# lab-incert/peba1

Measured on AMD Instinct MI355X. Metric: bootstrapped gates/sec (blind rotations/s) over the PEBA1 match path, and end-to-end match ms, higher is better.
Workload: dtype u32

## Files before the change

peba1_amd/csrc/kernels.hip:

```cpp
#include <type_traits>

#include "kernels.hpp"
#include "ntt_wave.hpp"

namespace tfhe_hip {

namespace {

__device__ __forceinline__ PrimeCtx make_ctx(int q, const uint32_t *tw, int n_ring) {
    PrimeCtx c;
    c.P = q ? NTT_P1 : NTT_P0;
    c.pinv = q ? NTT_PINV1 : NTT_PINV0;
    c.rmod = q ? NTT_R[1] : NTT_R[0];
    c.wf = tw + (size_t)(q * 2 + 0) * n_ring;
    c.wi = tw + (size_t)(q * 2 + 1) * n_ring;
    const uint4 *quads = reinterpret_cast<const uint4 *>(tw + (size_t)4 * n_ring);
    c.qf = quads + (size_t)(q * 2 + 0) * (n_ring / 2);
    c.qi = quads + (size_t)(q * 2 + 1) * (n_ring / 2);
    c.dtab = nullptr;
    c.fw1 = nullptr;
    c.fw2 = nullptr;
    return c;
}

__device__ __forceinline__ PrimeCtx make_sub_ctx(int q, int h, const uint32_t *tw, int n_ring) {
    return make_ctx(q, tw + (size_t)12 * n_ring + (size_t)h * 6 * n_ring, n_ring / 2);
}

template <int LOGN>
__device__ __forceinline__ void finish_inverse(const int64_t (&acc)[WaveNtt<LOGN>::REGS],
                                               int32_t (&y)[WaveNtt<LOGN>::REGS],
                                               const PrimeCtx &c, uint32_t *scr, int lane) {
    constexpr int REGS = WaveNtt<LOGN>::REGS;
#pragma unroll
    for (int r = 0; r < REGS; ++r) y[r] = mont_redc(acc[r], c.P, c.pinv);
    WaveNtt<LOGN>::inverse(y, c, scr, lane);
}

template <int LOGN>
__global__ __launch_bounds__(64) void bk_transform_kernel(const int32_t *__restrict__ raw, uint32_t *__restrict__ img,
                                                          const uint32_t *__restrict__ tw, int nw,
                                                          uint32_t scale0, uint32_t scale1) {
    using NTT = WaveNtt<LOGN>;
    constexpr int N = NTT::N, REGS = NTT::REGS;
    __shared__ __align__(16) uint32_t scr[NTT::SCRATCH_WORDS];
    const int lane = threadIdx.x;
    const int q = blockIdx.y;
    const int poly = blockIdx.x;
    const int X = poly / nw, w = poly % nw;
    const PrimeCtx c = make_ctx(q, tw, N);
    const uint32_t scale = q ? scale1 : scale0;
    const int32_t *src = raw + (size_t)poly * N;
    int32_t x[REGS];
#pragma unroll
    for (int r = 0; r < REGS; ++r) x[r] = src[r * 64 + lane] % (int32_t)c.P;
    NTT::forward(x, c, scr, lane);
    uint4 *dst = reinterpret_cast<uint4 *>(img + ((size_t)(X * 2 + q) * nw + w) * N) + lane;
#pragma unroll
    for (int g = 0; g < REGS / 4; ++g) {
        uint32_t v[4];
#pragma unroll
        for (int e = 0; e < 4; ++e) {
            int32_t m = x[4 * g + e] % (int32_t)c.P;
            if (m < 0) m += (int32_t)c.P;
            v[e] = (uint32_t)((uint64_t)(uint32_t)m * scale % c.P);
        }
        dst[g * 64] = make_uint4(v[0], v[1], v[2], v[3]);
    }
}

template <int LOGN>
__global__ __launch_bounds__(128) void negacyclic_kernel(const int32_t *__restrict__ ip, const uint32_t *__restrict__ img,
                                                         const uint32_t *__restrict__ tw, int32_t *__restrict__ res) {
    using NTT = WaveNtt<LOGN>;
    constexpr int N = NTT::N, REGS = NTT::REGS;
    __shared__ __align__(16) uint32_t lds_scr[2][NTT::SCRATCH_WORDS];
    const int tid = threadIdx.x;
    const int q = __builtin_amdgcn_readfirstlane(tid >> 6);
    const int lane = tid & 63;
    const PrimeCtx c = make_ctx(q, tw, N);
    uint32_t *scr = lds_scr[q];
    const int32_t *src = ip + (size_t)blockIdx.x * N;
    int32_t x[REGS];
#pragma unroll
    for (int r = 0; r < REGS; ++r) x[r] = src[r * 64 + lane];
    NTT::forward(x, c, scr, lane);
    const uint4 *bp = reinterpret_cast<const uint4 *>(img + (size_t)(blockIdx.x * 2 + q) * N) + lane;
    int64_t acc[REGS];
#pragma unroll
    for (int g = 0; g < REGS / 4; ++g) {
        const uint4 b = bp[g * 64];
        acc[4 * g + 0] = (int64_t)x[4 * g + 0] * (int32_t)b.x;
        acc[4 * g + 1] = (int64_t)x[4 * g + 1] * (int32_t)b.y;
        acc[4 * g + 2] = (int64_t)x[4 * g + 2] * (int32_t)b.z;
        acc[4 * g + 3] = (int64_t)x[4 * g + 3] * (int32_t)b.w;
    }
    int32_t y[REGS];
    finish_inverse<LOGN>(acc, y, c, scr, lane);
#pragma unroll
    for (int r = 0; r < REGS; ++r) scr[r * 64 + lane] = (uint32_t)y[r];
    __syncthreads();
    if (q == 0) {
        const uint32_t *oscr = lds_scr[1];
#pragma unroll
        for (int r = 0; r < REGS; ++r)
            res[(size_t)blockIdx.x * N + r * 64 + lane] = (int32_t)crt_signed_to_torus(y[r], (int32_t)oscr[r * 64 + lane]);
    }
}

template <int LOGN, int THREADS>
__device__ __forceinline__ void prelude_modswitch(const DevParams &p, const RotDesc &rd, const int32_t *__restrict__ pool,
                                                  uint16_t *lds_bar, int tid) {
    const int32_t *A = pool + (size_t)rd.slot_a * p.ct_stride;
    const int32_t *B = pool + (size_t)rd.slot_b * p.ct_stride;
    if (rd.slot_c < 0) {
        for (int i = tid; i <= p.n; i += THREADS) {
            uint32_t t = (uint32_t)rd.sa * (uint32_t)A[i] + (uint32_t)rd.sb * (uint32_t)B[i];
            if (i == p.n) t += (uint32_t)rd.c0;
            lds_bar[i] = (uint16_t)((t + (1u << (30 - LOGN))) >> (31 - LOGN));
        }
    } else {
        const int32_t *C = pool + (size_t)rd.slot_c * p.ct_stride;
        for (int i = tid; i <= p.n; i += THREADS) {
            uint32_t t = (uint32_t)rd.sa * (uint32_t)A[i] + (uint32_t)rd.sb * (uint32_t)B[i] + (uint32_t)rd.sc * (uint32_t)C[i];
            if (i == p.n) t += (uint32_t)rd.c0;
            lds_bar[i] = (uint16_t)((t + (1u << (30 - LOGN))) >> (31 - LOGN));
        }
    }
}

struct ClockProbe {
    unsigned long long c0 = 0, r0 = 0;
    bool on = false;
    __device__ __forceinline__ void begin(const DevParams &p) {
        on = p.clock_acc != nullptr && blockIdx.x % 61 == 0 && threadIdx.x == 0;
        if (on) { c0 = __builtin_amdgcn_s_memtime(); r0 = __builtin_amdgcn_s_memrealtime(); }
    }
    __device__ __forceinline__ void end(const DevParams &p) {
        if (on) {
            atomicAdd(&p.clock_acc[0], __builtin_amdgcn_s_memtime() - c0);
            atomicAdd(&p.clock_acc[1], __builtin_amdgcn_s_memrealtime() - r0);
        }
    }
};

template <int LOGN>
__device__ __forceinline__ uint32_t testvector_coef(int j, int barb, int32_t mu) {
    constexpr int N = 1 << LOGN;
    const int idx = (j + barb) & (2 * N - 1);
    return (idx & N) ? (uint32_t)(-mu) : (uint32_t)mu;
}

template <int LOGN>
__device__ __forceinline__ uint32_t lut_coef(const int32_t *__restrict__ v, int j, int barb) {
    constexpr int N = 1 << LOGN;
    const int idx = (j + barb) & (2 * N - 1);
    const uint32_t w = (uint32_t)v[idx & (N - 1)];
    return (idx & N) ? 0u - w : w;
}

__device__ __forceinline__ const int32_t *lut_of(const DevParams &p, const RotDesc &rd) {
    return rd.lut >= 0 ? p.luts + (size_t)rd.lut * LUT_STRIDE : nullptr;
}

template <int LOGN>
__device__ __forceinline__ uint32_t body_coef(const int32_t *__restrict__ lut, int j, int barb, int32_t mu) {
    return lut ? lut_coef<LOGN>(lut, j, barb) : testvector_coef<LOGN>(j, barb, mu);
}

template <int LOGN>
struct AccLds {
    static constexpr int N = 1 << LOGN;
    uint32_t w[2][3 * N];
    __device__ __forceinline__ void set(int u, int j, uint32_t v) {
        w[u][j] = v; w[u][N + j] = 0u - v; w[u][2 * N + j] = v;
    }
    __device__ __forceinline__ uint32_t get(int u, int j) const { return w[u][j]; }
    template <int REGS>
    __device__ __forceinline__ void rotated_difference(uint32_t (&D)[REGS], int u, int lane, int abar, uint32_t offset) const {
        const uint32_t base = (uint32_t)(lane - abar) & (uint32_t)(2 * N - 1);
        const uint32_t *own_neg = w[u] + N + lane;
        const uint32_t *rot = w[u] + base;
#pragma unroll
        for (int r = 0; r < REGS; ++r) D[r] = (rot[r * 64] + own_neg[r * 64] + offset) ^ offset;
    }
};

template <int LOGN, bool FRESH, bool TABLE, bool LDSTW = false, bool PROGRESS = false, int V = 0>
__device__ __forceinline__ void forward_poly(const DevParams &p, const DevKey &key, const PrimeCtx &c,
                                             const AccLds<LOGN> &lds_acc, uint32_t *scr,
                                             int lane, int q, int i, int u, int abar, bool swap_outputs,
                                             int64_t (&acc0)[WaveNtt<LOGN>::REGS], int64_t (&acc1)[WaveNtt<LOGN>::REGS],
                                             const typename WaveNtt<LOGN>::FwdTw0 &t0, int jbegin = 0, int jend = -1) {
    using NTT = WaveNtt<LOGN>;
    constexpr int N = NTT::N, REGS = NTT::REGS, G4 = REGS / 4;
    uint32_t Dk[REGS];
    lds_acc.template rotated_difference<REGS>(Dk, u, lane, abar, p.decomp_offset);
    const int o0 = swap_outputs ? N / 4 : 0, o1 = N / 4 - o0;
    const int width = p.Bgbit;
    auto row = [&](int jj, auto first) {
        const int prow = u * p.l + jj;
        const uint4 *bp = reinterpret_cast<const uint4 *>(
                              key.bk_img + ((size_t)((size_t)i * p.kpl + prow) * 2 + q) * 2 * N) + lane;
        uint4 b0[G4], b1[G4];
#pragma unroll
        for (int g = 0; g < G4; ++g) b0[g] = bp[o0 + g * 64];
#pragma unroll
        for (int g = 0; g < G4; ++g) b1[g] = bp[o1 + g * 64];
        const int shift = 32 - (jj + 1) * width;
        int32_t x[REGS];
        NTT::template forward_digits<TABLE, LDSTW>(x, Dk, shift, width, c, scr, lane, t0);
#pragma unroll
        for (int g = 0; g < G4; ++g) {
            const int32_t bb0[4] = {(int32_t)b0[g].x, (int32_t)b0[g].y, (int32_t)b0[g].z, (int32_t)b0[g].w};
#pragma unroll
            for (int e = 0; e < 4; ++e) {
                const int r = 4 * g + e;
                if constexpr (decltype(first)::value) acc0[r] = (int64_t)x[r] * bb0[e];
                else acc0[r] += (int64_t)x[r] * bb0[e];
            }
        }
#pragma unroll
        for (int g = 0; g < G4; ++g) {
            const int32_t bb1[4] = {(int32_t)b1[g].x, (int32_t)b1[g].y, (int32_t)b1[g].z, (int32_t)b1[g].w};
#pragma unroll
            for (int e = 0; e < 4; ++e) {
                const int r = 4 * g + e;
                if constexpr (decltype(first)::value) acc1[r] = (int64_t)x[r] * bb1[e];
                else acc1[r] += (int64_t)x[r] * bb1[e];
            }
        }
    };
    if (jend < 0) jend = p.l;
    row(jbegin, std::integral_constant<bool, FRESH>{});
#pragma unroll 1
    for (int jj = jbegin + 1; jj < jend; ++jj) {
        if constexpr (PROGRESS) {
            if (jj == jbegin + 1) __builtin_amdgcn_s_setprio(1);
            else __builtin_amdgcn_s_setprio(2);
        }
        row(jj, std::false_type{});
    }
}

template <int LOGN, int THREADS, typename AccT>
__device__ __forceinline__ void extract_sample(const DevParams &p, const RotDesc &rd,
                                               const AccT &acc,
                                               int32_t *__restrict__ u_buf, int32_t *__restrict__ acc_dbg, int tid) {
    constexpr int N = 1 << LOGN;
    int32_t *u = u_buf + (size_t)rd.u_index * p.u_stride;
    for (int j = tid; j < N; j += THREADS)
        u[j] = (int32_t)(j == 0 ? acc.get(0, 0) : 0u - acc.get(0, N - j));
    if (tid == 0) u[N] = (int32_t)acc.get(1, 0);
    if (acc_dbg) {
        int32_t *d = acc_dbg + (size_t)blockIdx.x * 2 * N;
        for (int j = tid; j < 2 * N; j += THREADS) d[j] = (int32_t)acc.get(j >> LOGN, j & (N - 1));
    }
}

template <int LOGN>
__global__ __launch_bounds__(128) void blind_rotate2_kernel(DevParams p, DevKey key, const int32_t *__restrict__ pool,
                                                           const RotDesc *__restrict__ rots,
                                                           int32_t *__restrict__ u_buf, int32_t *__restrict__ acc_dbg) {
    using NTT = WaveNtt<LOGN>;
    constexpr int N = NTT::N, REGS = NTT::REGS;
    __shared__ __align__(16) AccLds<LOGN> lds_acc;
    __shared__ __align__(16) uint32_t lds_scr[2][NTT::SCRATCH_WORDS];
    __shared__ uint16_t lds_bar[1024 + 8];

    const int tid = threadIdx.x;
    const int q = __builtin_amdgcn_readfirstlane(tid >> 6);
    const int lane = tid & 63;
    const PrimeCtx c = make_ctx(q, key.tw, N);
    uint32_t *scr = lds_scr[q];
    const RotDesc rd = rots[blockIdx.x];
    const int n = p.n;

    prelude_modswitch<LOGN, 128>(p, rd, pool, lds_bar, tid);
    __syncthreads();
    {
        const int barb = lds_bar[n];
        const int32_t *lut = lut_of(p, rd);
#pragma unroll
        for (int r = 0; r < REGS; ++r) {
            const int j = r * 64 + lane;
            lds_acc.set(q, j, q == 0 ? 0u : body_coef<LOGN>(lut, j, barb, p.mu));
        }
    }
    __syncthreads();

    typename NTT::FwdTw0 t0;
    t0.load(c, lane);
    for (int i = 0; i < n; ++i) {
        const int abar = __builtin_amdgcn_readfirstlane((int)lds_bar[i]);
        if (abar == 0) continue;

        int64_t acc0[REGS], acc1[REGS];
        forward_poly<LOGN, true, false>(p, key, c, lds_acc, scr, lane, q, i, 0, abar, false, acc0, acc1, t0);
        forward_poly<LOGN, false, false>(p, key, c, lds_acc, scr, lane, q, i, 1, abar, false, acc0, acc1, t0);

        int32_t y0[REGS], y1[REGS];
        finish_inverse<LOGN>(acc0, y0, c, scr, lane);
        finish_inverse<LOGN>(acc1, y1, c, scr, lane);

        const uint32_t *oscr = lds_scr[1 - q];
        if (q == 0) {
#pragma unroll
            for (int r = 0; r < REGS; ++r) scr[r * 64 + lane] = (uint32_t)y1[r];
            __syncthreads();
#pragma unroll
            for (int r = 0; r < REGS; ++r)
                lds_acc.set(0, r * 64 + lane, lds_acc.get(0, r * 64 + lane) + crt_signed_to_torus(y0[r], (int32_t)oscr[r * 64 + lane]));
        } else {
#pragma unroll
            for (int r = 0; r < REGS; ++r) scr[r * 64 + lane] = (uint32_t)y0[r];
            __syncthreads();
#pragma unroll
            for (int r = 0; r < REGS; ++r)
                lds_acc.set(1, r * 64 + lane, lds_acc.get(1, r * 64 + lane) + crt_signed_to_torus((int32_t)oscr[r * 64 + lane], y1[r]));
        }
        __syncthreads();
    }
    extract_sample<LOGN, 128>(p, rd, lds_acc, u_buf, acc_dbg, tid);
}

#ifdef TFHE_HIP_STAMPS
__device__ unsigned long long g_stamps[8][8];
#define STAMP_DECL unsigned long long st_prev = __builtin_amdgcn_s_memtime(), st_sum[8] = {0, 0, 0, 0, 0, 0, 0, 0}
#define STAMP(k)                                                             \
    do {                                                                     \
        __builtin_amdgcn_sched_barrier(0);                                   \
        const unsigned long long st_now = __builtin_amdgcn_s_memtime();      \
        __builtin_amdgcn_s_waitcnt(0xC07F);                                  \
        st_sum[k] += st_now - st_prev;                                       \
        st_prev = st_now;                                                    \
        __builtin_amdgcn_sched_barrier(0);                                   \
    } while (0)
#define STAMP_FLUSH                                                          \
    do {                                                                     \
        if (lane == 0)                                                       \
            for (int k = 0; k < 8; ++k) atomicAdd(&g_stamps[wv][k], st_sum[k]); \
    } while (0)
#else
#define STAMP_DECL
#define STAMP(k)
#define STAMP_FLUSH
#endif

template <int LOGN>
struct Br4Lds {
    using NTT = WaveNtt<LOGN>;
    AccLds<LOGN> acc;
    uint32_t buf0[4][NTT::SCRATCH_WORDS];
    uint32_t buf1[4][NTT::ROW_WORDS];
    uint16_t bar[1024 + 8];
    alignas(8) uint32_t dtab[2][5 * DIGIT_TAB];
    uint4 ft1[2][64 >> NTT::LC][NTT::FwdTw1::IMAGE16];
    uint4 ft2[2][64][NTT::FwdTw2::IMAGE16];
    __device__ __forceinline__ uint32_t *scr(int wv) { return buf0[wv]; }
    __device__ __forceinline__ uint32_t *x1(int wv) { return buf1[wv]; }
    __device__ __forceinline__ uint32_t *x2(int wv) { return buf0[wv]; }
};
static_assert(sizeof(Br4Lds<10>) <= 80 * 1024, "two workgroups of the 4-wave form must fit the 160 KB of a CU");

template <int LOGN, bool TAB, int V = 0>
__device__ __forceinline__ void blind_rotate4_body(const DevParams &p, const DevKey &key,
                                                   const int32_t *__restrict__ pool, const RotDesc &rd,
                                                   Br4Lds<LOGN> &sh, int tid) {
    using NTT = WaveNtt<LOGN>;
    constexpr int N = NTT::N, REGS = NTT::REGS, HALF = REGS / 2;
    const int wv = __builtin_amdgcn_readfirstlane(tid >> 6);
    const int q = wv & 1, u = wv >> 1;
    const int lane = tid & 63;
    PrimeCtx c = make_ctx(q, key.tw, N);
    uint32_t *scr = sh.scr(wv);
    const int n = p.n;

    prelude_modswitch<LOGN, 256>(p, rd, pool, sh.bar, tid);
    if constexpr (TAB) {
        NTT::build_digit_table(sh.dtab[q], c, p.Bgbit, (u << 6) | lane, 128);
        c.dtab = sh.dtab[q];
    }
    if (u == 0) {
        typename NTT::FwdTw1 a;
        a.load(c, lane);
        if ((lane & ((1 << NTT::LC) - 1)) == 0) a.to_image(sh.ft1[q][lane >> NTT::LC]);
        typename NTT::FwdTw2 b;
        b.load(c, lane);
        b.to_image(sh.ft2[q][lane]);
    }
    c.fw1 = sh.ft1[q][lane >> NTT::LC];
    c.fw2 = sh.ft2[q][lane];
    __syncthreads();
    if (q == 0) {
        const int barb = sh.bar[n];
        const int32_t *lut = lut_of(p, rd);
#pragma unroll
        for (int r = 0; r < REGS; ++r) {
            const int j = r * 64 + lane;
            sh.acc.set(u, j, u == 0 ? 0u : body_coef<LOGN>(lut, j, barb, p.mu));
        }
    }
    __syncthreads();

    STAMP_DECL;
    typename NTT::FwdTw0 t0;
    t0.load(c, lane);

    for (int i = 0; i < n; ++i) {
        const int abar = __builtin_amdgcn_readfirstlane((int)sh.bar[i]);
        if (abar == 0) continue;
        STAMP(0);

        int64_t acc0[REGS], acc1[REGS];
        forward_poly<LOGN, true, TAB, true, true, V>(p, key, c, sh.acc, scr, lane, q, i, u, abar, u != 0, acc0, acc1, t0);
        STAMP(1);

        int32_t t[REGS];
        {
            int32_t send[REGS];
#pragma unroll
            for (int r = 0; r < REGS; ++r) {
                t[r] = mont_redc(acc0[r], c.P, c.pinv);
                send[r] = mont_redc(acc1[r], c.P, c.pinv);
            }
            NTT::write_row(send, sh.x1(wv), lane);
        }
        typename NTT::InvTw2 t2;
        t2.load(c, lane);
        STAMP(2);
        lds_barrier();
        __builtin_amdgcn_s_setprio(3);
        STAMP(3);
        {
            int32_t other[REGS];
            NTT::read_row(other, sh.x1(wv ^ 2), lane);
#pragma unroll
            for (int r = 0; r < REGS; ++r) t[r] += other[r];
        }
        NTT::inverse(t, c, scr, lane, t2);
        STAMP(4);

        const uint32_t *ox = sh.x2(wv ^ 1);
        uint32_t *mx = sh.x2(wv);
        if (q == 0) {
#pragma unroll
            for (int r = 0; r < HALF; ++r) mx[r * 64 + lane] = (uint32_t)t[HALF + r];
            LDS_BARRIER_ROLE("q=0");
#pragma unroll
            for (int r = 0; r < HALF; ++r)
                sh.acc.set(u, r * 64 + lane, sh.acc.get(u, r * 64 + lane) + crt_signed_to_torus(t[r], (int32_t)ox[r * 64 + lane]));
        } else {
#pragma unroll
            for (int r = 0; r < HALF; ++r) mx[r * 64 + lane] = (uint32_t)t[r];
            LDS_BARRIER_ROLE("q=1");
#pragma unroll
            for (int r = 0; r < HALF; ++r)
                sh.acc.set(u, (HALF + r) * 64 + lane,
                           sh.acc.get(u, (HALF + r) * 64 + lane) + crt_signed_to_torus((int32_t)ox[r * 64 + lane], t[HALF + r]));
        }
        STAMP(5);
        __builtin_amdgcn_s_setprio(0);
        lds_barrier();
        STAMP(6);
    }
    STAMP_FLUSH;
}

template <int LOGN, bool TAB>
__global__ __launch_bounds__(256, 2) void blind_rotate4_kernel(
    DevParams p, DevKey key, const int32_t *__restrict__ pool, const RotDesc *__restrict__ rots,
    int32_t *__restrict__ u_buf, int32_t *__restrict__ acc_dbg) {
    __shared__ __align__(16) Br4Lds<LOGN> sh;
    if (p.wg_times && threadIdx.x == 0) {
        const uint64_t hw = __builtin_amdgcn_s_getreg((31 << 11) | (0 << 6) | 4);
        const uint64_t xcc = __builtin_amdgcn_s_getreg((3 << 11) | (0 << 6) | 20);
        p.wg_times[4 * blockIdx.x] = (__builtin_amdgcn_s_memtime() & 0xFFFFFFFFFFFFull) |
                                     ((((xcc & 0xF) << 8) | ((hw >> 8) & 0xFF)) << 48);
        p.wg_times[4 * blockIdx.x + 2] = __builtin_amdgcn_s_memrealtime();
    }
    ClockProbe clk;
    clk.begin(p);
    const RotDesc rd = rots[blockIdx.x];
    blind_rotate4_body<LOGN, TAB>(p, key, pool, rd, sh, threadIdx.x);
    extract_sample<LOGN, 256>(p, rd, sh.acc, u_buf, acc_dbg, threadIdx.x);
    clk.end(p);
    if (p.wg_times && threadIdx.x == 0) {
        p.wg_times[4 * blockIdx.x + 1] = __builtin_amdgcn_s_memtime();
        p.wg_times[4 * blockIdx.x + 3] = __builtin_amdgcn_s_memrealtime();
    }
}

__device__ __forceinline__ uint32_t split_finish(int h, int32_t a0, int32_t a1, int32_t b0, int32_t b1, uint32_t iw1_0,
                                                 uint32_t iw1_1) {
    if (h == 0) return crt_signed_to_torus(a0 + a1, b0 + b1);
    return crt_signed_to_torus(mont_mul(a0 - a1, iw1_0, NTT_P0, NTT_PINV0), mont_mul(b0 - b1, iw1_1, NTT_P1, NTT_PINV1));
}

template <int LOGN>
struct Br8Lds {
    using NTT = WaveNtt<LOGN>;
    AccLds<LOGN> acc;
    static_assert(WaveNtt<LOGN - 1>::SCRATCH_WORDS <= NTT::ROW_WORDS, "the half transform's scratch fits the full-size rows");
    uint32_t scr[8][NTT::ROW_WORDS];
    uint32_t pa0[4][NTT::ROW_WORDS];
    uint32_t pa1[4][NTT::ROW_WORDS];
    uint32_t pb0[4][NTT::ROW_WORDS];
    uint32_t pb[4][NTT::ROW_WORDS];
    uint16_t bar[1024 + 8];
    alignas(8) uint32_t dtab[2][5 * DIGIT_TAB];
    uint4 ft1[2][64 >> NTT::LC][NTT::FwdTw1::IMAGE16];
    uint4 ft2[2][64][NTT::FwdTw2::IMAGE16];
};

template <int LOGN, bool TAB>
__global__ __launch_bounds__(512, 2) void blind_rotate8_kernel(
    DevParams p, DevKey key, const int32_t *__restrict__ pool, const RotDesc *__restrict__ rots,
    int32_t *__restrict__ u_buf, int32_t *__restrict__ acc_dbg) {
    __shared__ __align__(16) Br8Lds<LOGN> sh;
#define BR8_TAG 0
#include "br8_body.inc"
#undef BR8_TAG
}

template <int LOGN, bool TAB>
__global__ __launch_bounds__(256, 2) void blind_rotate4_mk_kernel(
    DevParams p, DevKey key, const DevKey *__restrict__ keys, const int32_t *__restrict__ rot_keys,
    const int32_t *__restrict__ pool, const RotDesc *__restrict__ rots, int32_t *__restrict__ u_buf) {
    __shared__ __align__(16) Br4Lds<LOGN> sh;
    ClockProbe clk;
    clk.begin(p);
    const RotDesc rd = rots[blockIdx.x];
    DevKey k = key;
    k.bk_img = keys[__builtin_amdgcn_readfirstlane(rot_keys[blockIdx.x])].bk_img;
    blind_rotate4_body<LOGN, TAB, 1>(p, k, pool, rd, sh, threadIdx.x);
    extract_sample<LOGN, 256>(p, rd, sh.acc, u_buf, nullptr, threadIdx.x);
    clk.end(p);
}

template <int LOGN, bool TAB>
__global__ __launch_bounds__(512, 2) void blind_rotate8_mk_kernel(
    DevParams p, DevKey key, const DevKey *__restrict__ keys, const int32_t *__restrict__ rot_keys,
    const int32_t *__restrict__ pool, const RotDesc *__restrict__ rots, int32_t *__restrict__ u_buf) {
    __shared__ __align__(16) Br8Lds<LOGN> sh;
    int32_t *const acc_dbg = nullptr;
    {
        const DevKey key0 = key;
        DevKey key = key0;
        key.bk_img = keys[__builtin_amdgcn_readfirstlane(rot_keys[blockIdx.x])].bk_img;
#define BR8_TAG 1
#include "br8_body.inc"
#undef BR8_TAG
    }
}

constexpr int SPLIT_TAB2_BITS = 6;
template <int LOGN, int TM>
struct BrSplitLds {
    using SUB = WaveNtt<LOGN - 1>;
    AccLds<LOGN> acc;
    uint32_t scr[8][SUB::SCRATCH_WORDS];
    uint32_t x1[8][SUB::ROW_WORDS];
    uint16_t bar[1024 + 8];
    alignas(8) uint32_t tab[2][2][TM == 2 ? 11 << SPLIT_TAB2_BITS : DIGIT_TAB];
    static constexpr bool LTW = LOGN == 11;
    uint4 ft1[LTW ? 2 : 1][LTW ? 2 : 1][LTW ? (64 >> SUB::LC) : 1][SUB::FwdTw1::IMAGE16];
    uint4 ft2[LTW ? 2 : 1][LTW ? 2 : 1][LTW ? 64 : 1][SUB::FwdTw2::IMAGE16];
};
static_assert(sizeof(BrSplitLds<11, 2>) <= 160 * 1024, "the N = 2048 split form must fit a CU's LDS");

template <int LOGN, int TM>
__global__ __launch_bounds__(512, (LOGN == 10 ? 4 : 2)) void blind_rotate_split_kernel(
    DevParams p, DevKey key, const int32_t *__restrict__ pool, const RotDesc *__restrict__ rots,
    int32_t *__restrict__ u_buf, int32_t *__restrict__ acc_dbg) {
    using SUB = WaveNtt<LOGN - 1>;
    constexpr int N = 1 << LOGN, M = N / 2, RS = SUB::REGS, RF = 2 * RS, G4 = RS / 4, QUARTER = RS / 4;
    __shared__ __align__(16) BrSplitLds<LOGN, TM> sh;
    constexpr bool TAB = TM == 1;
    const int tid = threadIdx.x;
    const int wv = __builtin_amdgcn_readfirstlane(tid >> 6);
    const int q = wv & 1, u = (wv >> 1) & 1, h = wv >> 2;
    const int lane = tid & 63;
    PrimeCtx c = make_sub_ctx(q, h, key.tw, N);
    constexpr bool LTW = BrSplitLds<LOGN, TM>::LTW;
    uint32_t *scr = sh.scr[wv];
    const int n = p.n;
    const RotDesc rd = rots[blockIdx.x];
    const uint32_t w1 = key.tw[(size_t)(q * 2 + 0) * N + 1];
    const uint32_t iw1_0 = key.tw[(size_t)1 * N + 1], iw1_1 = key.tw[(size_t)3 * N + 1];
    ClockProbe clk;
    clk.begin(p);

    prelude_modswitch<LOGN, 512>(p, rd, pool, sh.bar, tid);
    if constexpr (TAB) {
        const int fields = 1 << p.Bgbit;
        for (int f = (u << 6) | lane; f < fields; f += 128) {
            const int32_t d = f < fields / 2 ? f : f - fields;
            const int32_t v = mont_mul(d, w1, c.P, c.pinv);
            sh.tab[q][h][f] = (uint32_t)(h ? -v : v);
        }
    }
    if constexpr (LTW) {
        if (u == 0) {
            typename SUB::FwdTw1 a;
            a.load(c, lane);
            if ((lane & ((1 << SUB::LC) - 1)) == 0) a.to_image(sh.ft1[q][h][lane >> SUB::LC]);
            typename SUB::FwdTw2 b;
            b.load(c, lane);
            b.to_image(sh.ft2[q][h][lane]);
        }
        c.fw1 = sh.ft1[q][h][lane >> SUB::LC];
        c.fw2 = sh.ft2[q][h][lane];
    }
    if constexpr (TM == 2) {
        const uint4 qd = c.qf[1];
        const uint32_t cst[6] = {0u, c.wf[1], qd.x, qd.z, qd.y, qd.w};
        const int fields = 1 << p.Bgbit;
        for (int e = (u << 6) | lane; e < 11 * fields; e += 128) {
            const int k = e / fields, f = e - k * fields;
            const int32_t d = f < fields / 2 ? f : f - fields;
            const bool hi = k == 0 || (k & 1) == 0;
            int32_t v = d;
            if (hi) { v = mont_mul(v, w1, c.P, c.pinv); if (h) v = -v; }
            if (k > 0) v = mont_mul(v, cst[(k + 1) >> 1], c.P, c.pinv);
            const int32_t half = (int32_t)(c.P >> 1);
            if (v > half) v -= (int32_t)c.P;
            if (v < -half) v += (int32_t)c.P;
            const int pos = k < 3 ? (k << SPLIT_TAB2_BITS) + f
                                  : ((3 + 2 * ((k - 3) & 3)) << SPLIT_TAB2_BITS) + 2 * f + (k >= 7 ? 1 : 0);
            sh.tab[q][h][pos] = (uint32_t)v;
        }
    }
    __syncthreads();
    if (q == 0) {
        const int barb = sh.bar[n];
        const int32_t *lut = lut_of(p, rd);
#pragma unroll
        for (int r = 0; r < RS; ++r) {
            const int j = h * M + r * 64 + lane;
            sh.acc.set(u, j, u == 0 ? 0u : body_coef<LOGN>(lut, j, barb, p.mu));
        }
    }
    __syncthreads();

    const int width = p.Bgbit;
    const int lane_off = G4 * (lane & 1) * 64 + h * 32 + (lane >> 1);
    const int o0 = u ? N / 4 : 0, o1 = N / 4 - o0;
    typename SUB::FwdTw0 t0;
    t0.load(c, lane);
    for (int i = 0; i < n; ++i) {
        const int abar = __builtin_amdgcn_readfirstlane((int)sh.bar[i]);
        if (abar == 0) continue;
        uint32_t D[RF];
        sh.acc.template rotated_difference<RF>(D, u, lane, abar, p.decomp_offset);
        int64_t acc0[RS], acc1[RS];
        auto row = [&](int jj, auto first) {
            const int prow = u * p.l + jj;
            const uint4 *bp = reinterpret_cast<const uint4 *>(
                                  key.bk_img + ((size_t)((size_t)i * p.kpl + prow) * 2 + q) * 2 * N) + lane_off;
            uint4 b0[G4], b1[G4];
#pragma unroll
            for (int g = 0; g < G4; ++g) b0[g] = bp[o0 + g * 64];
#pragma unroll
            for (int g = 0; g < G4; ++g) b1[g] = bp[o1 + g * 64];
            const int shift = 32 - (jj + 1) * width;
            int32_t x[RS];
            if constexpr (TM == 2) {
                constexpr int RBIT = SUB::rbit_of(0), hb = 1 << RBIT, lb = hb >> 1;
                const uint32_t mask4 = ((1u << width) - 1u) << 2;
                const int sh2 = shift - 2;
                const char *tab = reinterpret_cast<const char *>(sh.tab[q][h]);
                auto entry = [&](int k, uint32_t off) {
                    return (int32_t)*reinterpret_cast<const uint32_t *>(tab + (k << (SPLIT_TAB2_BITS + 2)) + off);
                };
                auto field = [&](int i) { return (D[i] >> sh2) & mask4; };
                const uint32_t mask8 = mask4 << 1;
                const int sh3 = shift - 3;
                auto pair = [&](int k, uint32_t off) {
                    return *reinterpret_cast<const uint2 *>(tab + ((3 + 2 * (k - 3)) << (SPLIT_TAB2_BITS + 2)) + off);
                };
                auto field8 = [&](int i) { return (D[i] >> sh3) & mask8; };
#pragma unroll
                for (int r = 0; r < RS; ++r)
                    if (!(r & (hb | lb))) {
                        const uint32_t l2 = field(r | hb), h0 = field(RS + r), h2 = field(RS + (r | hb));
                        const uint2 pl1 = pair(3, field8(r | lb)), ph1 = pair(4, field8(RS + (r | lb)));
                        const uint2 pl3 = pair(5, field8(r | hb | lb)), ph3 = pair(6, field8(RS + (r | hb | lb)));
                        const int32_t x0 = __builtin_amdgcn_sbfe((int32_t)D[r], shift, width) + entry(0, h0);
                        const int32_t A = entry(1, l2) + entry(2, h2);
                        const int32_t S = ((int32_t)pl1.x + (int32_t)ph1.x) + ((int32_t)pl3.x + (int32_t)ph3.x);
                        const int32_t T = ((int32_t)pl1.y + (int32_t)ph1.y) + ((int32_t)pl3.y + (int32_t)ph3.y);
                        const int32_t uu = x0 + A, vv = x0 - A;
                        x[r] = uu + S; x[r | lb] = uu - S; x[r | hb] = vv + T; x[r | hb | lb] = vv - T;
                    }
            } else if constexpr (TAB) {
                const uint32_t mask4 = ((1u << width) - 1u) << 2;
                const int sh2 = shift - 2;
                const char *tab = reinterpret_cast<const char *>(sh.tab[q][h]);
#pragma unroll
                for (int r = 0; r < RS; ++r)
                    x[r] = __builtin_amdgcn_sbfe((int32_t)D[r], shift, width) +
                           (int32_t)*reinterpret_cast<const uint32_t *>(tab + ((D[r + RS] >> sh2) & mask4));
            } else {
#pragma unroll
                for (int r = 0; r < RS; ++r) {
                    const int32_t v = mont_mul(__builtin_amdgcn_sbfe((int32_t)D[r + RS], shift, width), w1, c.P, c.pinv);
                    x[r] = __builtin_amdgcn_sbfe((int32_t)D[r], shift, width) + (h ? -v : v);
                }
            }
            if constexpr (TM == 2) SUB::template forward_rest<LTW>(x, c, scr, lane, t0);
            else SUB::template forward<LTW>(x, c, scr, lane, t0);
#pragma unroll
            for (int g = 0; g < G4; ++g) {
                const int32_t bb0[4] = {(int32_t)b0[g].x, (int32_t)b0[g].y, (int32_t)b0[g].z, (int32_t)b0[g].w};
                const int32_t bb1[4] = {(int32_t)b1[g].x, (int32_t)b1[g].y, (int32_t)b1[g].z, (int32_t)b1[g].w};
#pragma unroll
                for (int e = 0; e < 4; ++e) {
                    const int r = 4 * g + e;
// ... 534 lines not shown
```

Before: 108,700.

## Prefetch next bootstrapping-key row across blind-rotation steps

Adds a forward_poly variant that loads the first key half (k0) for the next decomposition row, or for the first row of the next non-skipped step, while the current row's multiply-accumulate is still running. The main loop now walks non-zero abar steps ahead of time so the next step index is known in advance. The aim is to hide global-memory latency on bootstrapping-key loads behind the NTT digit and MAC work. The cost is extra live vector registers for the carried k0 buffer, which could reduce occupancy or cause spills.

```diff
diff --git a/peba1_amd/csrc/kernels.hip b/peba1_amd/csrc/kernels.hip
--- a/peba1_amd/csrc/kernels.hip
+++ b/peba1_amd/csrc/kernels.hip
@@ -239,6 +239,71 @@
             if (jj == jbegin + 1) __builtin_amdgcn_s_setprio(1);
             else __builtin_amdgcn_s_setprio(2);
         }
+        row(jj, std::false_type{});
+    }
+}
+
+struct KeyRowWalk {
+    const uint32_t *img;
+    int i, inext, n;
+};
+
+template <int LOGN, bool TABLE, int V = 0>
+__device__ __forceinline__ void forward_poly_ahead(const DevParams &p, const KeyRowWalk &w, const PrimeCtx &c,
+                                                   const AccLds<LOGN> &lds_acc, uint32_t *scr,
+                                                   int lane, int q, int u, int abar, bool swap_outputs,
+                                                   int64_t (&acc0)[WaveNtt<LOGN>::REGS], int64_t (&acc1)[WaveNtt<LOGN>::REGS],
+                                                   uint4 (&k0)[WaveNtt<LOGN>::REGS / 4],
+                                                   const typename WaveNtt<LOGN>::FwdTw0 &t0) {
+    using NTT = WaveNtt<LOGN>;
+    constexpr int N = NTT::N, REGS = NTT::REGS, G4 = REGS / 4;
+    uint32_t Dk[REGS];
+    lds_acc.template rotated_difference<REGS>(Dk, u, lane, abar, p.decomp_offset);
+    const int o0 = swap_outputs ? N / 4 : 0, o1 = N / 4 - o0;
+    const int width = p.Bgbit, l = p.l;
+    auto tile = [&](int step, int jj) {
+        return reinterpret_cast<const uint4 *>(w.img + ((size_t)((size_t)step * p.kpl + u * l + jj) * 2 + q) * 2 * N) + lane;
+    };
+    auto row = [&](int jj, auto first) {
+        uint4 k1[G4];
+        const uint4 *bp = tile(w.i, jj);
+#pragma unroll
+        for (int g = 0; g < G4; ++g) k1[g] = bp[o1 + g * 64];
+        const int shift = 32 - (jj + 1) * width;
+        int32_t x[REGS];
+        NTT::template forward_digits<TABLE, true>(x, Dk, shift, width, c, scr, lane, t0);
+#pragma unroll
+        for (int g = 0; g < G4; ++g) {
+            const int32_t bb0[4] = {(int32_t)k0[g].x, (int32_t)k0[g].y, (int32_t)k0[g].z, (int32_t)k0[g].w};
+#pragma unroll
+            for (int e = 0; e < 4; ++e) {
+                const int r = 4 * g + e;
+                if constexpr (decltype(first)::value) acc0[r] = (int64_t)x[r] * bb0[e];
+                else acc0[r] += (int64_t)x[r] * bb0[e];
+            }
+        }
+        const bool last = jj + 1 == l;
+        const uint4 *np = tile(last ? (w.inext < w.n ? w.inext : w.i) : w.i, last ? 0 : jj + 1);
+        __builtin_amdgcn_sched_barrier(0);
+#pragma unroll
+        for (int g = 0; g < G4; ++g) k0[g] = np[o0 + g * 64];
+        __builtin_amdgcn_sched_barrier(0);
+#pragma unroll
+        for (int g = 0; g < G4; ++g) {
+            const int32_t bb1[4] = {(int32_t)k1[g].x, (int32_t)k1[g].y, (int32_t)k1[g].z, (int32_t)k1[g].w};
+#pragma unroll
+            for (int e = 0; e < 4; ++e) {
+                const int r = 4 * g + e;
+                if constexpr (decltype(first)::value) acc1[r] = (int64_t)x[r] * bb1[e];
+                else acc1[r] += (int64_t)x[r] * bb1[e];
+            }
+        }
+    };
+    row(0, std::true_type{});
+#pragma unroll 1
+    for (int jj = 1; jj < l; ++jj) {
+        if (jj == 1) __builtin_amdgcn_s_setprio(1);
+        else __builtin_amdgcn_s_setprio(2);
         row(jj, std::false_type{});
     }
 }
@@ -407,13 +472,25 @@
     typename NTT::FwdTw0 t0;
     t0.load(c, lane);
 
-    for (int i = 0; i < n; ++i) {
-        const int abar = __builtin_amdgcn_readfirstlane((int)sh.bar[i]);
-        if (abar == 0) continue;
+    auto next_step = [&](int i) {
+        do ++i; while (i < n && __builtin_amdgcn_readfirstlane((int)sh.bar[i]) == 0);
+        return i;
+    };
+    KeyRowWalk w{key.bk_img, next_step(-1), 0, n};
+    uint4 k0[REGS / 4];
+    if (w.i < n) {
+        const uint4 *bp = reinterpret_cast<const uint4 *>(
+                              key.bk_img + ((size_t)((size_t)w.i * p.kpl + u * p.l) * 2 + q) * 2 * N) + lane;
+#pragma unroll
+        for (int g = 0; g < REGS / 4; ++g) k0[g] = bp[(u != 0 ? N / 4 : 0) + g * 64];
+    }
+    for (; w.i < n; w.i = w.inext) {
+        const int abar = __builtin_amdgcn_readfirstlane((int)sh.bar[w.i]);
+        w.inext = next_step(w.i);
         STAMP(0);
 
         int64_t acc0[REGS], acc1[REGS];
-        forward_poly<LOGN, true, TAB, true, true, V>(p, key, c, sh.acc, scr, lane, q, i, u, abar, u != 0, acc0, acc1, t0);
+        forward_poly_ahead<LOGN, TAB, V>(p, w, c, sh.acc, scr, lane, q, u, abar, u != 0, acc0, acc1, k0, t0);
         STAMP(1);
 
         int32_t t[REGS];
```

After: 105,000. 0.966x the previous value.
